# MartinMikkelsen/TensorTrainNumerics.jl

Measured on AMD Instinct MI355X. Metric: TT cores/sec for QTT Laplacian apply+round, d=30 rank-64, higher is better.
Workload: dtype f64

## Files before the change

### include/ttn.h

```cpp
#ifndef TTN_H
#define TTN_H

#include <stdint.h>

#ifdef __cplusplus
extern "C" {
#endif

#define TTN_OK                 0
#define TTN_ERR_DIMS          -1
#define TTN_ERR_BOND_INDEX    -2
#define TTN_ERR_SWEEPS        -3
#define TTN_ERR_CENTER        -4
#define TTN_ERR_CAPACITY      -5
#define TTN_ERR_ARG           -6
#define TTN_ERR_NOT_INIT      -7
#define TTN_ERR_UNSUPPORTED   -8
#define TTN_ERR_NO_CONVERGENCE -9
#define TTN_ERR_SINGULAR      -10

int         ttn_init(int device);
int         ttn_finalize(void);
const char* ttn_version(void);
const char* ttn_last_error_string(void);
// ... 120 lines not shown
int ttn_dot_pullback(ttn_tt_t a, ttn_tt_t b, const double* delta, ttn_tt_t abar, ttn_tt_t bbar, double* out);
int ttn_apply_pullback(ttn_tto_t A, ttn_tt_t x, ttn_tt_t ybar, ttn_tt_t xbar);
int ttn_tt_cores_axpby(const double* alpha, ttn_tt_t x, const double* beta, ttn_tt_t y);
int ttn_tt_cores_dot(ttn_tt_t x, ttn_tt_t y, double* out);

int ttn_hadamard(ttn_tt_t x, ttn_tt_t y, ttn_tt_t z);
int ttn_add(ttn_tt_t x, ttn_tt_t y, ttn_tt_t z);
int ttn_scale(double a, ttn_tt_t x, ttn_tt_t y);
int ttn_scale_batch(const double* a, ttn_tt_t x, ttn_tt_t y);
int ttn_orthogonalize(ttn_tt_t x, int64_t center, ttn_tt_t y);

int ttn_sv_capture(ttn_tt_t h, int enable);
int ttn_sv_get(ttn_tt_t h, int64_t b, int64_t step, double* out, int64_t cap, int64_t* n);

int ttn_timer_begin(void);
int ttn_timer_end(float* ms);
int ttn_event_record(int64_t slot);
int ttn_event_elapsed(int64_t slot_a, int64_t slot_b, float* ms);

int ttn_selftest_gemm(int64_t m, int64_t n, int64_t k, const double* A, const double* B, double* C, double alpha, double beta,
                      int ta, int tb);

int ttn_selftest_eig128(const double* G, int64_t n, int64_t r, int64_t nev, double* sig, double* X, int64_t* ticks_rc);
int ttn_selftest_sym_eig(int64_t N, int64_t k, const double* A, double* lam, double* Y);
int ttn_debug_ortho_state(int64_t b, int64_t* out4);

int ttn_apply_f64(int64_t d, const int64_t* dims,
                  const double* const* A_cores, const int64_t* A_rks,
                  const double* const* X_cores, const int64_t* X_rks,
                  double* const* Y_cores);
int ttn_dot_f64(int64_t d, const int64_t* dims,
                const double* const* A_cores, const int64_t* A_rks,
                const double* const* B_cores, const int64_t* B_rks, double* out);
int ttn_hadamard_f64(int64_t d, const int64_t* dims,
                     const double* const* X_cores, const int64_t* X_rks,
                     const double* const* Y_cores, const int64_t* Y_rks,
                     double* const* Z_cores);
int ttn_add_f64(int64_t d, const int64_t* dims,
                const double* const* X_cores, const int64_t* X_rks,
                const double* const* Y_cores, const int64_t* Y_rks,
                double* const* Z_cores);
int ttn_scale_f64(int64_t d, const int64_t* dims, double a,
                  const double* const* X_cores, const int64_t* X_rks, const int64_t* X_ot,
                  double* const* Y_cores, int64_t* Y_ot);
int ttn_orthogonalize_f64(int64_t d, const int64_t* dims,
                          const double* const* X_cores, const int64_t* X_rks, int64_t center,
// ... 48 lines not shown
```

### tensortrainnumerics.jl_amd/_lib.py

```python
from __future__ import annotations

import ctypes as C
import os
import subprocess

_HERE = os.path.dirname(os.path.abspath(__file__))
LIB_PATH = os.environ.get("TTN_LIB") or os.path.join(_HERE, "libttn_hip.so")
CSRC = os.path.join(_HERE, "csrc")
INCLUDE = os.path.join(os.path.dirname(_HERE), "include")

TTN_OK = 0
TTN_ERR_DIMS = -1
TTN_ERR_BOND_INDEX = -2
TTN_ERR_SWEEPS = -3
TTN_ERR_CENTER = -4
TTN_ERR_CAPACITY = -5
TTN_ERR_ARG = -6
TTN_ERR_NOT_INIT = -7
TTN_ERR_UNSUPPORTED = -8
TTN_ERR_NO_CONVERGENCE = -9
TTN_ERR_SINGULAR = -10

i64 = C.c_int64
p_i64 = C.POINTER(C.c_int64)
# ... 70 lines not shown
    "ttn_dmrg_linsolve": (C.c_int, [handle, handle, handle, handle, C.c_double, i64, p_i64, p_i64]),
    "ttn_dmrg_linsolve_it": (C.c_int, [handle, handle, handle, handle, C.c_double, i64, p_i64, p_i64, C.c_int, i64, C.c_double, i64]),
    "ttn_dmrg_cg_iterations": (C.c_int, [i64, p_i64]),
    "ttn_dmrg_eigsolve": (C.c_int, [handle, handle, handle, C.c_double, i64, p_i64, p_i64, C.c_int, i64, C.c_double, i64, i64, p_f64, p_i64]),
    "ttn_mals_eigsolve": (C.c_int, [handle, handle, handle, C.c_double, i64, p_i64, p_i64, C.c_int, i64, C.c_double, i64, i64, p_f64, p_i64]),
    "ttn_eigsolve_history_len": (C.c_int, [C.c_int, i64, i64, p_i64, p_i64]),
    "ttn_als_eigsolve": (C.c_int, [handle, handle, handle, i64, p_i64, p_i64, p_f64, i64, C.c_int, i64, C.c_double, i64, i64, p_f64]),
    "ttn_als_gen_eigsolve": (C.c_int, [handle, handle, handle, handle, i64, p_i64, p_i64, C.c_int, i64, i64, p_f64]),
    "ttn_eigsolve_stats": (C.c_int, [i64, p_i64, p_f64]),
    "ttn_tdvp_apply_h1": (C.c_int, [C.c_int, i64, i64, i64, i64, i64, i64, C.c_void_p, C.c_void_p, C.c_void_p, C.c_void_p, C.c_void_p, C.c_int]),
    "ttn_tdvp_apply_h0": (C.c_int, [C.c_int, i64, i64, i64, i64, C.c_void_p, C.c_void_p, C.c_void_p, C.c_void_p]),
    "ttn_tdvp_update_left_env": (C.c_int, [C.c_int, i64, i64, i64, i64, i64, i64, C.c_void_p, C.c_void_p, C.c_void_p, C.c_void_p, C.c_int]),
    "ttn_tdvp_update_right_env": (C.c_int, [C.c_int, i64, i64, i64, i64, i64, i64, C.c_void_p, C.c_void_p, C.c_void_p, C.c_void_p, C.c_int]),
    "ttn_tdvp_apply_h2": (C.c_int, [C.c_int, i64, i64, i64, i64, i64, i64, i64, i64, C.c_void_p, C.c_void_p, C.c_void_p, C.c_void_p, C.c_void_p, C.c_void_p, C.c_int]),
    "ttn_dense_qr": (C.c_int, [C.c_int, i64, i64, C.c_void_p, C.c_void_p, C.c_void_p]),
    "ttn_dense_svd": (C.c_int, [C.c_int, i64, i64, C.c_void_p, C.c_void_p, C.c_void_p, C.c_void_p]),
    "ttn_cross_maxvol": (C.c_int, [C.c_int, i64, i64, C.c_void_p, C.c_double, i64, C.c_void_p, C.c_void_p, C.c_void_p, p_i64]),
    "ttn_cross_points": (C.c_int, [C.c_int, C.c_int, i64, i64, i64, i64, i64, i64, C.c_void_p, C.c_void_p, C.c_void_p, i64, C.c_void_p,
                                   C.c_void_p, C.c_void_p, C.c_void_p]),
    "ttn_cross_eval": (C.c_int, [C.c_int, i64, i64, pp_f64, p_i64, p_i64, C.c_void_p, C.c_void_p, C.c_void_p, C.c_void_p, C.c_double,
                                 C.c_void_p]),
    "ttn_tdvp_contract_f64": (C.c_int, [C.c_int, C.c_int, i64, p_i64, C.c_void_p, C.c_void_p, C.c_void_p, C.c_void_p, C.c_void_p, C.c_void_p, C.c_int]),
    "ttn_selftest_eig128": (C.c_int, [C.c_void_p, i64, i64, i64, C.c_void_p, C.c_void_p, C.c_void_p]),
    "ttn_selftest_sym_eig": (C.c_int, [i64, i64, C.c_void_p, C.c_void_p, C.c_void_p]),
    "ttn_add": (C.c_int, [handle, handle, handle]),
    "ttn_scale": (C.c_int, [C.c_double, handle, handle]),
    "ttn_scale_batch": (C.c_int, [p_f64, handle, handle]),
    "ttn_orthogonalize": (C.c_int, [handle, i64, handle]),
    "ttn_sv_capture": (C.c_int, [handle, C.c_int]),
    "ttn_sv_get": (C.c_int, [handle, i64, i64, p_f64, i64, p_i64]),
    "ttn_timer_begin": (C.c_int, []),
    "ttn_timer_end": (C.c_int, [C.POINTER(C.c_float)]),
    "ttn_selftest_gemm": (C.c_int, [i64, i64, i64, p_f64, p_f64, p_f64, C.c_double, C.c_double, C.c_int, C.c_int]),
    "ttn_event_record": (C.c_int, [i64]),
    "ttn_event_elapsed": (C.c_int, [i64, i64, C.POINTER(C.c_float)]),
    "ttn_apply_f64": (C.c_int, [i64, p_i64, pp_f64, p_i64, pp_f64, p_i64, pp_f64]),
    "ttn_dot_f64": (C.c_int, [i64, p_i64, pp_f64, p_i64, pp_f64, p_i64, p_f64]),
    "ttn_hadamard_f64": (C.c_int, [i64, p_i64, pp_f64, p_i64, pp_f64, p_i64, pp_f64]),
    "ttn_add_f64": (C.c_int, [i64, p_i64, pp_f64, p_i64, pp_f64, p_i64, pp_f64]),
    "ttn_scale_f64": (C.c_int, [i64, p_i64, C.c_double, pp_f64, p_i64, p_i64, pp_f64, p_i64]),
    "ttn_orthogonalize_f64": (C.c_int, [i64, p_i64, pp_f64, p_i64, i64, pp_f64, p_i64, p_i64]),
    "ttn_compress_f64": (C.c_int, [i64, p_i64, pp_f64, p_i64, i64, C.c_double, i64]),
    "ttn_apply_compress_rank_bound": (C.c_int, [i64, p_i64, p_i64, p_i64, i64, i64, p_i64]),
    "ttn_apply_compress_f64": (C.c_int, [i64, p_i64, pp_f64, p_i64, pp_f64, p_i64, pp_f64, p_i64, i64, C.c_double, i64]),
    "ttn_bond_truncate_f64": (C.c_int, [i64, p_i64, pp_f64, p_i64, i64, i64, C.c_double]),
    "ttn_r_and_d_to_rks": (C.c_int, [i64, p_i64, i64, p_i64, i64, p_i64]),
# ... 121 lines not shown
```

### tensortrainnumerics.jl_amd/csrc/ttn_api.hip

```cpp
#include "../../include/ttn.h"
#include "ttn_common.h"
#include "ttn_stream_kernels.h"
#include "ttn_dense_kernels.h"
#include "ttn_dot_kernels.h"
#include "ttn_ortho_kernels.h"
#include "ttn_ortho512.h"
#include "ttn_ortho_ramp.h"
#include "ttn_hsvd_kernels.h"
#include "ttn_resite_kernels.h"
#include "ttn_als_kernels.h"
#include "ttn_als_grid.h"
#include "ttn_eigsolve_kernels.h"
#include "ttn_als_eig_kernels.h"
#include "ttn_eig_kernels.h"
#include "ttn_tdvp_kernels.h"
#include "ttn_densefact_kernels.h"
#include "ttn_cross_kernels.h"
#include "ttn_cross_batch_kernels.h"
#include "ttn_opalg_kernels.h"
#include "ttn_cplx_kernels.h"
#include "ttn_grid_kernels.h"
#include "ttn_grad_kernels.h"
#include "ttn_rect_kernels.h"
#include "ttn_step_kernels.h"

#include <algorithm>
#include <cmath>
#include <cstdio>
#include <cstring>
#include <cstdlib>
#include <mutex>
#include <set>
#include <string>
#include <vector>

extern "C" {
int ttn_wg512_init(void);
size_t ttn_wg512_compress_args_bytes(void);
int ttn_wg512_launch_compress(const void* args, size_t nbytes, int grid, hipStream_t stream);
int ttn_wg512_selftest_eig(const double* G, double* Vst, int n, int r, int nev, double* sig, double* Xout, long long* clk, hipStream_t stream);
int ttn_wg512_selftest_gemm(int m, int n, int k, double* A, double* B, double* C, double alpha, double beta, int ta, int tb, hipStream_t stream);
}

namespace {
std::set<struct ttn_tt_s*> g_live;
std::recursive_mutex g_mu;
bool g_init = false;
int g_device = -1;
hipStream_t g_stream = nullptr;
hipEvent_t g_ev0 = nullptr, g_ev1 = nullptr;
hipEvent_t g_launch_ev0 = nullptr, g_launch_ev1 = nullptr;
bool g_have_launch_ms = false;
size_t g_ortho_state_off = 0;
int g_ortho_state_batch = 0;
long long g_dense_plan[3] = {-1, 0, 0};
long long g_gather_plan[4] = {0, 0, 0, 0};
std::string g_err = "";
std::vector<hipEvent_t> g_slots;
std::vector<long long> g_xb_tab_host;
hipEvent_t g_xb_tab_ev = nullptr;

int fail(int code, const char* what) {
    g_err = what;
// ... 146 lines not shown

const char* ttn_version(void) { return "ttn-mi355x 0.1.0 (gfx950, fp64)"; }
const char* ttn_last_error_string(void) { return g_err.c_str(); }

int ttn_device_count(int* n) {
    if (!n) return fail(TTN_ERR_ARG, "null pointer");
    int c = 0;
    hipError_t e = hipGetDeviceCount(&c);
    if (e != hipSuccess) { *n = 0; return hipfail(e, "hipGetDeviceCount"); }
    *n = c;
    return TTN_OK;
}

int ttn_init(int device) {
    std::lock_guard<std::recursive_mutex> lk(g_mu);
    if (g_init && device == g_device) return TTN_OK;
    if (g_init) return fail(TTN_ERR_ARG, "ttn_init: already bound to another device (call ttn_finalize first)");
    HIPCHK(hipSetDevice(device));
    HIPCHK(hipStreamCreateWithFlags(&g_stream, hipStreamNonBlocking));
    for (hipEvent_t* e : {&g_ev0, &g_ev1, &g_launch_ev0, &g_launch_ev1}) HIPCHK(hipEventCreate(e));
    const struct { const void* fn; size_t lds; } lds_limits[] = {
        {(const void*)k_compress, COMPRESS_LDS_BYTES},
        {(const void*)k_selftest_eig128, COMPRESS_LDS_BYTES},
        {(const void*)k_mals_linsolve, COMPRESS_LDS_BYTES},
        {(const void*)k_als_linsolve, COMPRESS_LDS_BYTES},
        {(const void*)k_two_site_eig, COMPRESS_LDS_BYTES},
        {(const void*)k_als_eig, COMPRESS_LDS_BYTES},
        {(const void*)k_increase_ranks, COMPRESS_LDS_BYTES},
        {(const void*)k_ttv_decomp, COMPRESS_LDS_BYTES},
        {(const void*)k_split_sites, COMPRESS_LDS_BYTES},
        {(const void*)k_swap_chain, COMPRESS_LDS_BYTES},
        {(const void*)k_orthogonalize, ORTHO_LDS_BYTES},
        {(const void*)k_ortho512, O5_LDS_BYTES(TTN_MAX_D * 8)},
        {(const void*)k_dot_fused, DOT_LDS_BYTES(DOT_MAX_D)},
        {(const void*)k_grad_chain, DOT_LDS_BYTES(DOT_MAX_D)},
        {(const void*)k_selftest_gemm, sizeof(double) * GEMM_LDS_TOTAL},
        {(const void*)k_tdvp, TDVP_LDS_BYTES},
        {(const void*)k_lu_panel, LU_PANEL_LDS_BYTES},
        {(const void*)k_lu_trail, sizeof(double) * GEMM_LDS_TOTAL},
        {(const void*)k_cross_maxvol<false>, TTN_XV_LDS_BYTES},
        {(const void*)k_cross_maxvol<true>, TTN_XV_LDS_BYTES},
        {(const void*)k_zcompress, TTN_ZC_LDS_BYTES},
        {(const void*)k_cross_batch_site, TTN_XB_LDS_BYTES},
    };
    for (const auto& a : lds_limits) HIPCHK(hipFuncSetAttribute(a.fn, hipFuncAttributeMaxDynamicSharedMemorySize, (int)a.lds));
    { const int rc512 = ttn_wg512_init(); if (rc512) return hipfail((hipError_t)rc512, "ttn_wg512_init"); }
// ... 2401 lines not shown
    NEED_INIT();
    if (!A || !B || !C || m < 1 || n < 1 || k < 1) return fail(TTN_ERR_ARG, "bad argument");
    double *dA = nullptr, *dB = nullptr, *dC = nullptr;
    HIPCHK(hipMalloc((void**)&dA, sizeof(double) * m * k));
    HIPCHK(hipMalloc((void**)&dB, sizeof(double) * k * n));
    HIPCHK(hipMalloc((void**)&dC, sizeof(double) * m * n));
    HIPCHK(hipMemcpyAsync(dA, A, sizeof(double) * m * k, hipMemcpyHostToDevice, g_stream));
    HIPCHK(hipMemcpyAsync(dB, B, sizeof(double) * k * n, hipMemcpyHostToDevice, g_stream));
    HIPCHK(hipMemcpyAsync(dC, C, sizeof(double) * m * n, hipMemcpyHostToDevice, g_stream));
    if (getenv("TTN_WG512_SELFTEST") && atoi(getenv("TTN_WG512_SELFTEST"))) {
        const int rc512 = ttn_wg512_selftest_gemm((int)m, (int)n, (int)k, dA, dB, dC, alpha, beta, ta, tb, g_stream);
        if (rc512) return hipfail((hipError_t)rc512, "k_selftest_gemm (512-thread build)");
    } else {
    hipLaunchKernelGGL(k_selftest_gemm, dim3(1), dim3(TTN_WG), sizeof(double) * GEMM_LDS_TOTAL, g_stream, (int)m, (int)n, (int)k,
                       dA, dB, dC, alpha, beta, ta, tb);
    HIPCHK(hipGetLastError());
    }
    HIPCHK(hipMemcpyAsync(C, dC, sizeof(double) * m * n, hipMemcpyDeviceToHost, g_stream));
    HIPCHK(hipStreamSynchronize(g_stream));
    hipFree(dA); hipFree(dB); hipFree(dC);
    return TTN_OK;
}

int ttn_selftest_eig128(const double* G, int64_t n, int64_t r, int64_t nev, double* sig, double* X, int64_t* ticks_rc) {
    std::lock_guard<std::recursive_mutex> lk(g_mu);
    NEED_INIT();
    if (!G || !sig || !X || (n != 64 && n != 128) || r < 1 || r > 64 || nev < r || nev > n) return fail(TTN_ERR_ARG, "bad argument");
    double *dG = nullptr, *dV = nullptr, *dS = nullptr, *dX = nullptr;
    long long* dC = nullptr;
    HIPCHK(hipMalloc((void**)&dG, sizeof(double) * 128 * 128));
    HIPCHK(hipMalloc((void**)&dV, sizeof(double) * 128 * 128));
    HIPCHK(hipMalloc((void**)&dS, sizeof(double) * 128));
    HIPCHK(hipMalloc((void**)&dX, sizeof(double) * 128 * 64));
    HIPCHK(hipMalloc((void**)&dC, sizeof(long long) * 2));
    HIPCHK(hipMemcpyAsync(dG, G, sizeof(double) * n * n, hipMemcpyHostToDevice, g_stream));
    HIPCHK(hipMemsetAsync(dX, 0, sizeof(double) * 128 * 64, g_stream));
    if (getenv("TTN_WG512_SELFTEST") && atoi(getenv("TTN_WG512_SELFTEST"))) {
        const int rc512 = ttn_wg512_selftest_eig(dG, dV, (int)n, (int)r, (int)nev, dS, dX, dC, g_stream);
        if (rc512) return hipfail((hipError_t)rc512, "k_selftest_eig128 (512-thread build)");
    } else {
    hipLaunchKernelGGL(k_selftest_eig128, dim3(1), dim3(TTN_WG), COMPRESS_LDS_BYTES, g_stream, dG, dV, (int)n, (int)r, (int)nev, dS, dX, dC);
    HIPCHK(hipGetLastError());
    }
    long long hc[2] = {0, 0};
    HIPCHK(hipMemcpyAsync(sig, dS, sizeof(double) * nev, hipMemcpyDeviceToHost, g_stream));
    HIPCHK(hipMemcpyAsync(X, dX, sizeof(double) * 128 * r, hipMemcpyDeviceToHost, g_stream));
    HIPCHK(hipMemcpyAsync(hc, dC, sizeof(hc), hipMemcpyDeviceToHost, g_stream));
    HIPCHK(hipStreamSynchronize(g_stream));
    if (ticks_rc) { ticks_rc[0] = hc[0]; ticks_rc[1] = hc[1]; }
    hipFree(dG); hipFree(dV); hipFree(dS); hipFree(dX); hipFree(dC);
    return TTN_OK;
}

int ttn_selftest_sym_eig(int64_t N, int64_t k, const double* A, double* lam, double* Y) {
    std::lock_guard<std::recursive_mutex> lk(g_mu);
    if (!A || !lam || !Y || N < 1 || N > TTN_DENSE_LOCAL_MAX || k < 1 || k > std::min<int64_t>(N, TTN_NWAVES))
        return fail(TTN_ERR_ARG, "ttn_selftest_sym_eig: need 1 <= N <= 2048 and 1 <= k <= min(N, 16)");
    NEED_INIT();
    double *dA = nullptr, *dL = nullptr, *dY = nullptr, *dW = nullptr;
    HIPCHK(hipMalloc((void**)&dA, sizeof(double) * N * N));
    HIPCHK(hipMalloc((void**)&dL, sizeof(double) * k));
    HIPCHK(hipMalloc((void**)&dY, sizeof(double) * N * k));
    HIPCHK(hipMalloc((void**)&dW, sizeof(double) * (3 * N + 5 * N * k)));
    HIPCHK(hipMemcpyAsync(dA, A, sizeof(double) * N * N, hipMemcpyHostToDevice, g_stream));
    HIPCHK(hipMemsetAsync(dY, 0, sizeof(double) * N * k, g_stream));
    hipLaunchKernelGGL(k_selftest_sym_eig, dim3(1), dim3(TTN_WG), 0, g_stream, (int)N, (int)k, dA, dL, dY, dW);
    HIPCHK(hipGetLastError());
    HIPCHK(hipMemcpyAsync(lam, dL, sizeof(double) * k, hipMemcpyDeviceToHost, g_stream));
    HIPCHK(hipMemcpyAsync(Y, dY, sizeof(double) * N * k, hipMemcpyDeviceToHost, g_stream));
    HIPCHK(hipStreamSynchronize(g_stream));
    hipFree(dA); hipFree(dL); hipFree(dY); hipFree(dW);
    return TTN_OK;
}

// ... 1218 lines not shown
```

### tensortrainnumerics.jl_amd/csrc/ttn_eig_kernels.h

```cpp
#pragma once
#include "ttn_dense_kernels.h"

#define EIG_N 128
template <int J>
__device__ __forceinline__ void fmac_bcast(double& a, double w, double s_) {
    asm volatile("v_fmac_f64_dpp %0, %1, %2 row_newbcast:%3 row_mask:0xf bank_mask:0xf" : "+v"(a) : "v"(w), "v"(s_), "n"(J));
}
#define EIG_BCAST16(M) M(0) M(1) M(2) M(3) M(4) M(5) M(6) M(7) M(8) M(9) M(10) M(11) M(12) M(13) M(14) M(15)
#define EIG_TAIL TTN_LDS_IMG

__device__ __forceinline__ void lds_barrier() { asm volatile("s_waitcnt lgkmcnt(0)\n\ts_barrier" ::: "memory"); }
__device__ __forceinline__ double wave64_sum_mfma(double v) {
    v = grp_sum(v);
    v += dpp_mov_f64<0x124>(v);
    v += dpp_mov_f64<0x128>(v);
    return v;
}
__device__ __forceinline__ double readlane_f64(double v, int idx) {
    union { double d; int i[2]; } u, r;
    u.d = v;
    r.i[0] = __builtin_amdgcn_readlane(u.i[0], idx);
    r.i[1] = __builtin_amdgcn_readlane(u.i[1], idx);
    return r.d;
}
// ... 100 lines not shown
            const double nvi = -vL[i], nwi = -wL[i];
            asm volatile("s_nop 1");
#define EIG_UP(j) fmac_bcast<j>(a[j], wreg[0], nvi); fmac_bcast<j>(a[j], vreg[0], nwi);
            EIG_BCAST16(EIG_UP)
#undef EIG_UP
            if constexpr (NH == 2) {
#define EIG_UP(j) fmac_bcast<j>(a[16 + j], wreg[1], nvi); fmac_bcast<j>(a[16 + j], vreg[1], nwi);
                EIG_BCAST16(EIG_UP)
#undef EIG_UP
            }
            if (i == k + 2) {
#pragma unroll
                for (int j = 0; j < CW; ++j) xn_w[CW * c + j] = a[j];
            }
        }
    }
    __syncthreads();
    if (actv && i == N - 2 && c == NC - 1) { dg[N - 2] = a[CW - 2]; e[N - 2] = a[CW - 1]; }
    if (actv && i == N - 1 && c == NC - 1) { dg[N - 1] = a[CW - 1]; }
    __syncthreads();
}

template <int N>
__device__ __forceinline__ int sturm_count(const double (&dreg)[N / 16], const double (&ereg)[N / 16], double x, bool& zero) {
    double pc = 1.0, pp = 0.0;
    const double nx = -x, one = 1.0;
    int cnt = 0;
    bool z = false;
    unsigned int prev = 0;
#pragma unroll
    for (int g = 0; g < N / 16; ++g) {
        unsigned int bits = 0;
#define EIG_ST(j) {                                                                                               \
            double dmx = nx;                                                                                      \
            fmac_bcast<j>(dmx, dreg[g], one);                                         \
            double pn = dmx * pc;                                                                                 \
            fmac_bcast<j>(pn, ereg[g], pp);                        \
            z |= (pn == 0.0);                                                                                     \
            bits = __builtin_amdgcn_alignbit(bits, (unsigned int)(__double_as_longlong(pn) >> 32), 31);           \
            pp = pc; pc = pn; }
        EIG_BCAST16(EIG_ST)
#undef EIG_ST
        const unsigned int seq = (prev << 16) | (bits & 0xffffu);
        cnt += __popc((seq ^ (seq >> 1)) & 0xffffu);
        prev = bits & 1u;
        const double ap = fabs(pc);
        if (ap < 0x1p-400 || ap > 0x1p400) {
            const double sc = (ap < 1.0) ? 0x1p500 : 0x1p-500;
            pc *= sc; pp *= sc;
        }
    }
    zero = z;
    return cnt;
}
__device__ __noinline__ int sturm_count_guarded(const lds_f64* de, double x, int n) {
    double pc = 1.0, pp = 0.0;
    int cnt = 0;
    for (int i = 0; i < n; ++i) {
        double pn = fma(de[2 * i] - x, pc, de[2 * i + 1] * pp);
        if (pn == 0.0) pn = copysign(DBL_MIN, -pc);
        cnt += (int)(((unsigned long long)(__double_as_longlong(pn) ^ __double_as_longlong(pc))) >> 63);
        pp = pc; pc = pn;
        const double ap = fabs(pc);
        if (ap < 0x1p-400 || ap > 0x1p400) { const double sc = (ap < 1.0) ? 0x1p500 : 0x1p-500; pc *= sc; pp *= sc; }
    }
    return cnt;
}

template <int N, int TL>
__device__ void wg_bisect(int nev, double* lds) {
    lds_f64* L = (lds_f64*)lds;
    lds_f64 *dg = L + EIG_TAIL, *e = dg + 128, *lam = dg + 256;
    lds_f64* e2 = L;
    const int tid = threadIdx.x;
    lds_f64* de = L + 256;
    for (int t = tid; t < N; t += TTN_WG) { e2[t] = (t < N - 1) ? e[t] * e[t] : 0.0; de[2 * t] = dg[t]; de[2 * t + 1] = (t > 0) ? -(e[t - 1] * e[t - 1]) : 0.0; }
    __syncthreads();
    if (tid < 64) {
        double glo_ = 1e300, ghi_ = -1e300, emax_ = 0.0;
        for (int t = tid; t < N; t += 64) {
            const double rad = ((t > 0) ? fabs(e[t - 1]) : 0.0) + ((t < N - 1) ? fabs(e[t]) : 0.0);
            glo_ = fmin(glo_, dg[t] - rad); ghi_ = fmax(ghi_, dg[t] + rad);
            emax_ = fmax(emax_, e2[t]);
        }
        glo_ = -wave_max(-glo_); ghi_ = wave_max(ghi_); emax_ = wave_max(emax_);
        if (tid == 0) { e2[128] = glo_; e2[129] = ghi_; e2[130] = emax_; }
    }
    __syncthreads();
    double glo = e2[128], ghi = e2[129];
    const double emax = e2[130];
    const double span = fmax(fabs(glo), fabs(ghi));
    glo -= 2.0 * DBL_EPSILON * span * N; ghi += 2.0 * DBL_EPSILON * span * N;
    const double pivmin = DBL_MIN * fmax(1.0, emax);
    double dreg[N / 16], ereg[N / 16];
#pragma unroll
    for (int g = 0; g < N / 16; ++g) { dreg[g] = de[2 * (16 * g + (tid & 15))]; ereg[g] = de[2 * (16 * g + (tid & 15)) + 1]; }
    asm volatile("s_nop 1");
    for (int g0 = 0; g0 < nev; g0 += TTN_WG / TL) {
        const int gi = g0 + tid / TL, sub = tid % TL;
        const bool act = gi < nev;
        const int jasc = N - 1 - (act ? gi : 0);
        double lo = glo, hi = ghi;
        for (int round = 0; round < 64; ++round) {
            const double wdt = hi - lo;
            const bool done = !(wdt > 2.0 * DBL_EPSILON * fmax(fabs(lo), fabs(hi)) + 2.0 * pivmin);
            if (__syncthreads_and(done || !act)) break;
            const double x = lo + wdt * ((double)(sub + 1) / (double)(TL + 1));
            const bool wave_act = g0 + (tid & ~63) / TL < nev;
            bool zero = false;
            int cnt = wave_act ? sturm_count<N>(dreg, ereg, x, zero) : 0;
            if (zero) cnt = sturm_count_guarded(de, x, N);
            int nf = (cnt <= jasc) ? 1 : 0;
#pragma unroll
            for (int m = 1; m < TL; m <<= 1) nf += __shfl_xor(nf, m);
            if (!done) {
                const double nlo = (nf > 0) ? lo + wdt * ((double)nf / (double)(TL + 1)) : lo;
                const double nhi = (nf < TL) ? lo + wdt * ((double)(nf + 1) / (double)(TL + 1)) : hi;
                lo = nlo; hi = nhi;
            }
        }
        if (act && sub == 0) lam[gi] = 0.5 * (lo + hi);
    }
    __syncthreads();
}

template <int N>
struct EigDm {
    static constexpr bool IN_LDS = 2 * N * 64 <= TTN_LDS_IMG;
    typedef __attribute__((address_space(1))) double gdouble;
    lds_f64* l;
    gdouble* g;
    __device__ __forceinline__ double ld(int idx) const { if constexpr (IN_LDS) return l[idx]; else return g[idx]; }
    __device__ __forceinline__ void st(int idx, double v) const { if constexpr (IN_LDS) l[idx] = v; else g[idx] = v; }
};
template <int N>
__device__ void wg_twisted(int r, double* lds, int* tw , lds_f64* zn , double* Dmg) {
    lds_f64* L = (lds_f64*)lds;
    lds_f64 *dg = L + EIG_TAIL, *e = dg + 128, *lam = dg + 256;
    lds_f64* Dp = L;
    EigDm<N> Dm;
    Dm.l = L + N * 64; Dm.g = (typename EigDm<N>::gdouble*)(unsigned long long)Dmg;
    const int tid = threadIdx.x, lane = tid & 63, wave = tid >> 6;
    double emax = 0.0;
    for (int t = 0; t < N - 1; ++t) emax = fmax(emax, e[t] * e[t]);
    const double pivmin = DBL_MIN * fmax(1.0, emax);
// ... 60 lines not shown
                for (int i0 = 0; i0 < N - 1; i0 += 8) {
                    double dm[8];
#pragma unroll
                    for (int t = 0; t < 8; ++t) dm[t] = (i0 + t + 1 < N) ? Dm.ld((i0 + t + 1) * 64 + lane) : 1.0;
#pragma unroll
                    for (int t = 0; t < 8; ++t) {
                        const int i = i0 + t;
                        if (i >= kb && i < N - 1) {
                            z = -(e[i] * fast_rcp(dm[t])) * z;
                            Dm.st((i + 1) * 64 + lane, z);
                            nrm = fma(z, z, nrm);
                        }
                    }
                }
            }
            if (act) zn[64 + lane] = nrm;
        }
    }
    __syncthreads();
    if (tid < 64 && tid < r) zn[tid] = 1.0 / sqrt(1.0 + zn[tid] + zn[64 + tid]);
    __syncthreads();
}

template <int N>
__device__ __noinline__ int wg_eig_n(const double* Gg, int ldg, double* Vst, int r, int nev, double* sig, double* lds, int* iwork ,
                                     double* dwork ) {
    Gg = unip(Gg); Vst = unip(Vst); sig = unip(sig); lds = unip(lds); iwork = unip(iwork); dwork = unip(dwork);
    r = uni32(r); nev = uni32(nev); ldg = uni32(ldg);
    constexpr int RPL = N / 16;
    lds_f64* L = (lds_f64*)lds;
    lds_f64 *lam = L + EIG_TAIL + 256, *beta = L + EIG_TAIL + 384;
    const int tid = threadIdx.x, lane = tid & 63, wave = tid >> 6;
    __builtin_amdgcn_s_setprio(TTN_EIG_PRIO);
    wg_tridiag<N>(Gg, ldg, Vst, lds);
    if (nev <= 32) wg_bisect<N, 8>(nev, lds);
    else wg_bisect<N, 4>(nev, lds);
    int bad = 0;
    for (int j = tid; j < nev; j += TTN_WG) { const double l = lam[j]; sig[j] = (l > 0.0) ? sqrt(l) : 0.0; bad |= (j < r) && !(l > 0.0); }
    if (__syncthreads_or(bad)) {
        __builtin_amdgcn_s_setprio(0); TTN_SETPRIO_BASE();
        return 1;
    }
    wg_twisted<N>(r, lds, iwork, (lds_f64*)dwork, const_cast<double*>(Gg));
    lds_f64* Dp = L;
    EigDm<N> Dm;
    Dm.l = L + N * 64; Dm.g = (typename EigDm<N>::gdouble*)(unsigned long long)Gg;
    const int rc = (lane & 3) | ((lane >> 4) << 2), col0 = 8 * (wave & 7) + 2 * ((lane >> 2) & 3);
    double z[2][RPL];
#pragma unroll
    for (int cc = 0; cc < 2; ++cc) {
        const int col = col0 + cc;
        const int kb = (col < r) ? iwork[col] : 0;
        const double zn = (col < r) ? ((lds_f64*)dwork)[col] : 0.0;
#pragma unroll
        for (int t = 0; t < RPL; ++t) {
            const int row = RPL * rc + t;
            const double v = (row < kb) ? Dp[row * 64 + col] : ((row == kb) ? 1.0 : Dm.ld(row * 64 + col));
            z[cc][t] = v * zn;
        }
// ... 35 lines not shown
        }
    }
    __syncthreads();
    __builtin_amdgcn_s_setprio(0); TTN_SETPRIO_BASE();
    return 0;
}
__device__ int wg_eig128(const double* Gg, double* Vst, int r, int nev, double* sig, double* lds, int* iwork, double* dwork) {
    return wg_eig_n<128>(Gg, 128, Vst, r, nev, sig, lds, iwork, dwork);
}
__device__ int wg_eig64(const double* Gg, int ldg, double* Vst, int r, int nev, double* sig, double* lds, int* iwork, double* dwork) {
    return wg_eig_n<64>(Gg, ldg, Vst, r, nev, sig, lds, iwork, dwork);
}

__global__ void TTN_KERNEL_BOUNDS k_selftest_eig128(const double* G, double* Vst, int n, int r, int nev, double* sig, double* Xout, long long* clk) {
    extern __shared__ double lds[];
    int* iwork = reinterpret_cast<int*>(lds + GEMM_LDS_TOTAL + 32);
    double* dwork = lds + GEMM_LDS_TOTAL + 32 + 64;
    const long long t0 = (long long)__builtin_amdgcn_s_memtime();
    const int rc = (n == 64) ? wg_eig_n<64>(G, 64, Vst, r, nev, sig, lds, iwork, dwork) : wg_eig_n<128>(G, 128, Vst, r, nev, sig, lds, iwork, dwork);
    const long long t1 = (long long)__builtin_amdgcn_s_memtime();
    if (threadIdx.x == 0) { clk[0] = t1 - t0; clk[1] = rc; }
    if (rc == 0) for (int e = threadIdx.x; e < 128 * r; e += TTN_WG) Xout[e] = lds[e];
}
```

### tensortrainnumerics.jl_amd/csrc/ttn_wg512.hip

```cpp
#include <hip/hip_runtime.h>
#include <stdint.h>
#include <float.h>
#include <string.h>

#define TTN_WG 512
namespace ttn_wg512 {
#include "ttn_common.h"
#include "ttn_dense_kernels.h"
#include "ttn_eig_kernels.h"
}

extern "C" {

int ttn_wg512_init(void) {
    hipError_t e;
    if ((e = hipFuncSetAttribute(reinterpret_cast<const void*>(ttn_wg512::k_compress), hipFuncAttributeMaxDynamicSharedMemorySize, (int)COMPRESS_LDS_BYTES)) != hipSuccess) return (int)e;
    if ((e = hipFuncSetAttribute(reinterpret_cast<const void*>(ttn_wg512::k_selftest_eig128), hipFuncAttributeMaxDynamicSharedMemorySize, (int)COMPRESS_LDS_BYTES)) != hipSuccess) return (int)e;
    if ((e = hipFuncSetAttribute(reinterpret_cast<const void*>(ttn_wg512::k_selftest_gemm), hipFuncAttributeMaxDynamicSharedMemorySize, (int)COMPRESS_LDS_BYTES)) != hipSuccess) return (int)e;
    return 0;
}

size_t ttn_wg512_compress_args_bytes(void) { return sizeof(ttn_wg512::CompressArgs); }
size_t ttn_wg512_lds_bytes(void) { return COMPRESS_LDS_BYTES; }

int ttn_wg512_launch_compress(const void* args, size_t nbytes, int grid, hipStream_t stream) {
    if (nbytes != sizeof(ttn_wg512::CompressArgs)) return (int)hipErrorInvalidValue;
    ttn_wg512::CompressArgs P;
    memcpy(&P, args, sizeof(P));
    hipLaunchKernelGGL(ttn_wg512::k_compress, dim3(grid), dim3(TTN_WG), COMPRESS_LDS_BYTES, stream, P);
    return (int)hipGetLastError();
}

int ttn_wg512_selftest_eig(const double* G, double* Vst, int n, int r, int nev, double* sig, double* Xout, long long* clk, hipStream_t stream) {
    hipLaunchKernelGGL(ttn_wg512::k_selftest_eig128, dim3(1), dim3(TTN_WG), COMPRESS_LDS_BYTES, stream, G, Vst, n, r, nev, sig, Xout, clk);
    return (int)hipGetLastError();
}
int ttn_wg512_selftest_gemm(int m, int n, int k, double* A, double* B, double* C, double alpha, double beta, int ta, int tb, hipStream_t stream) {
    hipLaunchKernelGGL(ttn_wg512::k_selftest_gemm, dim3(1), dim3(TTN_WG), COMPRESS_LDS_BYTES, stream, m, n, k, A, B, C, alpha, beta, ta, tb);
    return (int)hipGetLastError();
}

}
```

Measured before the change: 603,700.

## Accelerate tridiagonal bisection with coarse Sturm table and interpolated probe placement

The workgroup bisection eigensolver first evaluates a 256-point Sturm-count table over the Gershgorin interval. Each eigenvalue then starts from the bracketing table cell instead of the full interval. Within the bracket, probes are clustered around a secant or quadratic root estimate, built from the tracked mantissa and exponent of the Sturm recurrence's final pivot. A closing bisection replay reproduces the original bracket sequence and only calls Sturm counts where a probe falls inside the refined bracket, aiming to cut the number of Sturm passes in the SVD used by rounding. It also adds a statistics-collecting selftest kernel, at the cost of more register and LDS use and more complex control flow.

```diff
diff --git a/include/ttn.h b/include/ttn.h
--- a/include/ttn.h
+++ b/include/ttn.h
@@ -166,6 +166,7 @@
                       int ta, int tb);
 
 int ttn_selftest_eig128(const double* G, int64_t n, int64_t r, int64_t nev, double* sig, double* X, int64_t* ticks_rc);
+int ttn_selftest_eig128_ex(const double* G, int64_t n, int64_t r, int64_t nev, double* sig, double* X, int64_t* info);
 int ttn_selftest_sym_eig(int64_t N, int64_t k, const double* A, double* lam, double* Y);
 int ttn_debug_ortho_state(int64_t b, int64_t* out4);
 
diff --git a/tensortrainnumerics.jl_amd/_lib.py b/tensortrainnumerics.jl_amd/_lib.py
--- a/tensortrainnumerics.jl_amd/_lib.py
+++ b/tensortrainnumerics.jl_amd/_lib.py
@@ -116,6 +116,7 @@
                                  C.c_void_p]),
     "ttn_tdvp_contract_f64": (C.c_int, [C.c_int, C.c_int, i64, p_i64, C.c_void_p, C.c_void_p, C.c_void_p, C.c_void_p, C.c_void_p, C.c_void_p, C.c_int]),
     "ttn_selftest_eig128": (C.c_int, [C.c_void_p, i64, i64, i64, C.c_void_p, C.c_void_p, C.c_void_p]),
+    "ttn_selftest_eig128_ex": (C.c_int, [C.c_void_p, i64, i64, i64, C.c_void_p, C.c_void_p, C.c_void_p]),
     "ttn_selftest_sym_eig": (C.c_int, [i64, i64, C.c_void_p, C.c_void_p, C.c_void_p]),
     "ttn_add": (C.c_int, [handle, handle, handle]),
     "ttn_scale": (C.c_int, [C.c_double, handle, handle]),
diff --git a/tensortrainnumerics.jl_amd/csrc/ttn_api.hip b/tensortrainnumerics.jl_amd/csrc/ttn_api.hip
--- a/tensortrainnumerics.jl_amd/csrc/ttn_api.hip
+++ b/tensortrainnumerics.jl_amd/csrc/ttn_api.hip
@@ -39,6 +39,7 @@
 size_t ttn_wg512_compress_args_bytes(void);
 int ttn_wg512_launch_compress(const void* args, size_t nbytes, int grid, hipStream_t stream);
 int ttn_wg512_selftest_eig(const double* G, double* Vst, int n, int r, int nev, double* sig, double* Xout, long long* clk, hipStream_t stream);
+int ttn_wg512_selftest_eig_ex(const double* G, double* Vst, int n, int r, int nev, double* sig, double* Xout, long long* clk, hipStream_t stream);
 int ttn_wg512_selftest_gemm(int m, int n, int k, double* A, double* B, double* C, double alpha, double beta, int ta, int tb, hipStream_t stream);
 }
 
@@ -231,6 +232,7 @@
     const struct { const void* fn; size_t lds; } lds_limits[] = {
         {(const void*)k_compress, COMPRESS_LDS_BYTES},
         {(const void*)k_selftest_eig128, COMPRESS_LDS_BYTES},
+        {(const void*)k_selftest_eig128_ex, COMPRESS_LDS_BYTES},
         {(const void*)k_mals_linsolve, COMPRESS_LDS_BYTES},
         {(const void*)k_als_linsolve, COMPRESS_LDS_BYTES},
         {(const void*)k_two_site_eig, COMPRESS_LDS_BYTES},
@@ -2678,7 +2680,7 @@
     return TTN_OK;
 }
 
-int ttn_selftest_eig128(const double* G, int64_t n, int64_t r, int64_t nev, double* sig, double* X, int64_t* ticks_rc) {
+static int selftest_eig128_impl(const double* G, int64_t n, int64_t r, int64_t nev, double* sig, double* X, int64_t* words, int nwords) {
     std::lock_guard<std::recursive_mutex> lk(g_mu);
     NEED_INIT();
     if (!G || !sig || !X || (n != 64 && n != 128) || r < 1 || r > 64 || nev < r || nev > n) return fail(TTN_ERR_ARG, "bad argument");
@@ -2688,24 +2690,34 @@
     HIPCHK(hipMalloc((void**)&dV, sizeof(double) * 128 * 128));
     HIPCHK(hipMalloc((void**)&dS, sizeof(double) * 128));
     HIPCHK(hipMalloc((void**)&dX, sizeof(double) * 128 * 64));
-    HIPCHK(hipMalloc((void**)&dC, sizeof(long long) * 2));
+    HIPCHK(hipMalloc((void**)&dC, sizeof(long long) * 4));
     HIPCHK(hipMemcpyAsync(dG, G, sizeof(double) * n * n, hipMemcpyHostToDevice, g_stream));
     HIPCHK(hipMemsetAsync(dX, 0, sizeof(double) * 128 * 64, g_stream));
+    HIPCHK(hipMemsetAsync(dC, 0, sizeof(long long) * 4, g_stream));
+    const bool ex = nwords == 4;
     if (getenv("TTN_WG512_SELFTEST") && atoi(getenv("TTN_WG512_SELFTEST"))) {
-        const int rc512 = ttn_wg512_selftest_eig(dG, dV, (int)n, (int)r, (int)nev, dS, dX, dC, g_stream);
+        const int rc512 = ex ? ttn_wg512_selftest_eig_ex(dG, dV, (int)n, (int)r, (int)nev, dS, dX, dC, g_stream)
+                             : ttn_wg512_selftest_eig(dG, dV, (int)n, (int)r, (int)nev, dS, dX, dC, g_stream);
         if (rc512) return hipfail((hipError_t)rc512, "k_selftest_eig128 (512-thread build)");
     } else {
-    hipLaunchKernelGGL(k_selftest_eig128, dim3(1), dim3(TTN_WG), COMPRESS_LDS_BYTES, g_stream, dG, dV, (int)n, (int)r, (int)nev, dS, dX, dC);
-    HIPCHK(hipGetLastError());
-    }
-    long long hc[2] = {0, 0};
+    if (ex) hipLaunchKernelGGL(k_selftest_eig128_ex, dim3(1), dim3(TTN_WG), COMPRESS_LDS_BYTES, g_stream, dG, dV, (int)n, (int)r, (int)nev, dS, dX, dC);
+    else hipLaunchKernelGGL(k_selftest_eig128, dim3(1), dim3(TTN_WG), COMPRESS_LDS_BYTES, g_stream, dG, dV, (int)n, (int)r, (int)nev, dS, dX, dC);
+    HIPCHK(hipGetLastError());
+    }
+    long long hc[4] = {0, 0, 0, 0};
     HIPCHK(hipMemcpyAsync(sig, dS, sizeof(double) * nev, hipMemcpyDeviceToHost, g_stream));
     HIPCHK(hipMemcpyAsync(X, dX, sizeof(double) * 128 * r, hipMemcpyDeviceToHost, g_stream));
     HIPCHK(hipMemcpyAsync(hc, dC, sizeof(hc), hipMemcpyDeviceToHost, g_stream));
     HIPCHK(hipStreamSynchronize(g_stream));
-    if (ticks_rc) { ticks_rc[0] = hc[0]; ticks_rc[1] = hc[1]; }
+    if (words) for (int i = 0; i < nwords; ++i) words[i] = hc[i];
     hipFree(dG); hipFree(dV); hipFree(dS); hipFree(dX); hipFree(dC);
     return TTN_OK;
+}
+int ttn_selftest_eig128(const double* G, int64_t n, int64_t r, int64_t nev, double* sig, double* X, int64_t* ticks_rc) {
+    return selftest_eig128_impl(G, n, r, nev, sig, X, ticks_rc, 2);
+}
+int ttn_selftest_eig128_ex(const double* G, int64_t n, int64_t r, int64_t nev, double* sig, double* X, int64_t* info) {
+    return selftest_eig128_impl(G, n, r, nev, sig, X, info, 4);
 }
 
 int ttn_selftest_sym_eig(int64_t N, int64_t k, const double* A, double* lam, double* Y) {
diff --git a/tensortrainnumerics.jl_amd/csrc/ttn_eig_kernels.h b/tensortrainnumerics.jl_amd/csrc/ttn_eig_kernels.h
--- a/tensortrainnumerics.jl_amd/csrc/ttn_eig_kernels.h
+++ b/tensortrainnumerics.jl_amd/csrc/ttn_eig_kernels.h
@@ -146,10 +146,10 @@
 }
 
 template <int N>
-__device__ __forceinline__ int sturm_count(const double (&dreg)[N / 16], const double (&ereg)[N / 16], double x, bool& zero) {
+__device__ __forceinline__ int sturm_count(const double (&dreg)[N / 16], const double (&ereg)[N / 16], double x, bool& zero, double& mant, int& expo) {
     double pc = 1.0, pp = 0.0;
     const double nx = -x, one = 1.0;
-    int cnt = 0;
+    int cnt = 0, sh = 0;
     bool z = false;
     unsigned int prev = 0;
 #pragma unroll
@@ -170,11 +170,16 @@
         prev = bits & 1u;
         const double ap = fabs(pc);
         if (ap < 0x1p-400 || ap > 0x1p400) {
-            const double sc = (ap < 1.0) ? 0x1p500 : 0x1p-500;
+            const bool up = ap < 1.0;
+            const double sc = up ? 0x1p500 : 0x1p-500;
             pc *= sc; pp *= sc;
+            sh += up ? -500 : 500;
         }
     }
     zero = z;
+    int ex = 0;
+    mant = frexp(pc, &ex);
+    expo = sh + ex;
     return cnt;
 }
 __device__ __noinline__ int sturm_count_guarded(const lds_f64* de, double x, int n) {
@@ -191,13 +196,21 @@
     return cnt;
 }
 
-template <int N, int TL>
+#define EIG_NCOARSE 256
+#define EIG_FSTOP 8.0
+#define EIG_UNUSABLE (-(1 << 30))
+#define EIG_STATS_SLOT (EIG_TAIL + 511)
+template <int N, int TL, bool STATS>
 __device__ void wg_bisect(int nev, double* lds) {
     lds_f64* L = (lds_f64*)lds;
     lds_f64 *dg = L + EIG_TAIL, *e = dg + 128, *lam = dg + 256;
     lds_f64* e2 = L;
     const int tid = threadIdx.x;
     lds_f64* de = L + 256;
+    lds_f64* tm = L + 512;
+    lds_i32* tc = (lds_i32*)(L + 768);
+    lds_i32* te = (lds_i32*)(L + 896);
+    int* stats = (int*)(lds + EIG_STATS_SLOT);
     for (int t = tid; t < N; t += TTN_WG) { e2[t] = (t < N - 1) ? e[t] * e[t] : 0.0; de[2 * t] = dg[t]; de[2 * t + 1] = (t > 0) ? -(e[t - 1] * e[t - 1]) : 0.0; }
     __syncthreads();
     if (tid < 64) {
@@ -216,35 +229,164 @@
     const double span = fmax(fabs(glo), fabs(ghi));
     glo -= 2.0 * DBL_EPSILON * span * N; ghi += 2.0 * DBL_EPSILON * span * N;
     const double pivmin = DBL_MIN * fmax(1.0, emax);
+    const double gw = ghi - glo;
     double dreg[N / 16], ereg[N / 16];
 #pragma unroll
     for (int g = 0; g < N / 16; ++g) { dreg[g] = de[2 * (16 * g + (tid & 15))]; ereg[g] = de[2 * (16 * g + (tid & 15)) + 1]; }
     asm volatile("s_nop 1");
+    if (tid < EIG_NCOARSE) {
+        const double x = glo + gw * ((double)(tid + 1) / (double)(EIG_NCOARSE + 1));
+        bool zero = false;
+        double m;
+        int ex;
+        int cnt = sturm_count<N>(dreg, ereg, x, zero, m, ex);
+        if (zero) cnt = sturm_count_guarded(de, x, N);
+        if (zero || !(fabs(m) >= 0.5 && fabs(m) < 1.0)) ex = EIG_UNUSABLE;
+        tm[tid] = m; tc[tid] = cnt; te[tid] = ex;
+    }
+    __syncthreads();
+    auto tab_x = [&](int i) { return (i <= 0) ? glo : ((i > EIG_NCOARSE) ? ghi : glo + gw * ((double)i / (double)(EIG_NCOARSE + 1))); };
+    auto tab_c = [&](int i) { return (i <= 0) ? 0 : ((i > EIG_NCOARSE) ? N : tc[i - 1]); };
+    auto tab_e = [&](int i) { return (i <= 0 || i > EIG_NCOARSE) ? EIG_UNUSABLE : te[i - 1]; };
+    auto tab_m = [&](int i) { return (i <= 0 || i > EIG_NCOARSE) ? 0.0 : tm[i - 1]; };
+    const int sub = tid % TL;
+    const double frac = (double)(sub + 1) / (double)(TL + 1);
+    const int half = TL / 2, steps = (sub < half) ? half - 1 - sub : sub - half;
+    const double mult = ((sub < half) ? -1.0 : 1.0) * (double)(1 << ((TL == 4 ? 4 : 2) * steps));
     for (int g0 = 0; g0 < nev; g0 += TTN_WG / TL) {
-        const int gi = g0 + tid / TL, sub = tid % TL;
+        const int gi = g0 + tid / TL;
         const bool act = gi < nev;
         const int jasc = N - 1 - (act ? gi : 0);
-        double lo = glo, hi = ghi;
-        for (int round = 0; round < 64; ++round) {
+        int ta = 0, tb = EIG_NCOARSE + 1;
+#pragma unroll
+        for (int it = 0; it < 9; ++it) {
+            if (tb - ta > 1) {
+                const int mid = (ta + tb) >> 1;
+                if (tc[mid - 1] <= jasc) ta = mid; else tb = mid;
+            }
+        }
+        double lo = tab_x(ta), hi = tab_x(ta + 1), mlo = tab_m(ta), mhi = tab_m(ta + 1);
+        int clo = tab_c(ta), chi = tab_c(ta + 1), elo = tab_e(ta), ehi = tab_e(ta + 1);
+        double xo = 0.0, mo = 0.0;
+        int eo = EIG_UNUSABLE;
+        {
+            const int lt = (ta >= 1 && tab_e(ta - 1) != EIG_UNUSABLE) ? ta - 1 : -1;
+            const int rt = (ta + 2 <= EIG_NCOARSE + 1 && tab_e(ta + 2) != EIG_UNUSABLE) ? ta + 2 : -1;
+            const int pick = (lt >= 0 && (rt < 0 || tab_c(lt) == clo || tab_c(rt) != chi)) ? lt : rt;
+            if (pick >= 0) { xo = tab_x(pick); mo = tab_m(pick); eo = tab_e(pick); }
+        }
+        bool forced = false;
+        int myrounds = 1;
+        for (int round = 0; round < 128; ++round) {
             const double wdt = hi - lo;
-            const bool done = !(wdt > 2.0 * DBL_EPSILON * fmax(fabs(lo), fabs(hi)) + 2.0 * pivmin);
+            const double tolw = 2.0 * DBL_EPSILON * fmax(fabs(lo), fabs(hi)) + 2.0 * pivmin;
+            const bool done = !(wdt > EIG_FSTOP * tolw);
             if (__syncthreads_and(done || !act)) break;
-            const double x = lo + wdt * ((double)(sub + 1) / (double)(TL + 1));
-            const bool wave_act = g0 + (tid & ~63) / TL < nev;
+            double x = lo + wdt * frac;
+            bool placed = false;
+            if (!forced && chi - clo == 1 && elo != EIG_UNUSABLE && ehi != EIG_UNUSABLE && ((mlo < 0.0) != (mhi < 0.0))) {
+                int E = max(elo, ehi);
+                if (eo != EIG_UNUSABLE) E = max(E, eo);
+                const double flo = ldexp(mlo, max(elo - E, -2000)), fhi = ldexp(mhi, max(ehi - E, -2000));
+                const double s = lo + wdt * (flo * fast_rcp(flo - fhi));
+                double est = s, dqs = wdt;
+                if (eo != EIG_UNUSABLE) {
+                    const double fo = ldexp(mo, max(eo - E, -2000));
+                    const double whi = (flo * fo) * fast_rcp((fhi - flo) * (fhi - fo));
+                    const double wo = (flo * fhi) * fast_rcp((fo - flo) * (fo - fhi));
+                    const double q = lo + (wdt * whi + (xo - lo) * wo);
+                    if (q > lo && q < hi) est = q;
+                    dqs = fabs(q - s);
+                }
+                if (!(dqs < wdt)) dqs = wdt;
+                const double delta = fmin(fmax(2.0 * dqs, 0.5 * tolw), 0.125 * wdt);
+                const double c = est + mult * delta;
+                if (c > lo && c < hi) x = c;
+                placed = true;
+            }
+            const bool wave_act = __builtin_amdgcn_ballot_w64(act && !done) != 0ull;
             bool zero = false;
-            int cnt = wave_act ? sturm_count<N>(dreg, ereg, x, zero) : 0;
+            double m = 0.0;
+            int ex = EIG_UNUSABLE, cnt = 0;
+            if (wave_act) {
+                asm volatile("s_nop 1");
+                cnt = sturm_count<N>(dreg, ereg, x, zero, m, ex);
+                if constexpr (STATS) { if ((tid & 63) == 0) atomicAdd(stats + 1, 1); }
+            }
             if (zero) cnt = sturm_count_guarded(de, x, N);
-            int nf = (cnt <= jasc) ? 1 : 0;
-#pragma unroll
-            for (int m = 1; m < TL; m <<= 1) nf += __shfl_xor(nf, m);
+            if (zero || !(fabs(m) >= 0.5 && fabs(m) < 1.0)) ex = EIG_UNUSABLE;
+            double xl = -INFINITY, ml = 0.0, xr = INFINITY, mr = 0.0;
+            int el = EIG_UNUSABLE, er = EIG_UNUSABLE;
+            if (eo != EIG_UNUSABLE && xo < lo) { xl = xo; ml = mo; el = eo; }
+            if (eo != EIG_UNUSABLE && xo > hi) { xr = xo; mr = mo; er = eo; }
+            double nlo = lo, nmlo = mlo, nhi = hi, nmhi = mhi;
+            int nclo = clo, nelo = elo, nchi = chi, nehi = ehi;
+#pragma unroll
+            for (int t = 0; t < TL; ++t) {
+                const double xt = __shfl(x, t, TL), mt = __shfl(m, t, TL);
+                const int ct = __shfl(cnt, t, TL), et = __shfl(ex, t, TL);
+                if (ct <= jasc) {
+                    if (xt > nlo) { xl = nlo; ml = nmlo; el = nelo; nlo = xt; nclo = ct; nmlo = mt; nelo = et; }
+                    else if (xt > xl) { xl = xt; ml = mt; el = et; }
+                } else {
+                    if (xt < nhi) { xr = nhi; mr = nmhi; er = nehi; nhi = xt; nchi = ct; nmhi = mt; nehi = et; }
+                    else if (xt < xr) { xr = xt; mr = mt; er = et; }
+                }
+            }
             if (!done) {
-                const double nlo = (nf > 0) ? lo + wdt * ((double)nf / (double)(TL + 1)) : lo;
-                const double nhi = (nf < TL) ? lo + wdt * ((double)(nf + 1) / (double)(TL + 1)) : hi;
-                lo = nlo; hi = nhi;
-            }
-        }
-        if (act && sub == 0) lam[gi] = 0.5 * (lo + hi);
-    }
+                lo = nlo; clo = nclo; mlo = nmlo; elo = nelo; hi = nhi; chi = nchi; mhi = nmhi; ehi = nehi;
+                const bool left = el != EIG_UNUSABLE && (er == EIG_UNUSABLE || lo - xl <= xr - hi);
+                xo = left ? xl : xr; mo = left ? ml : mr; eo = left ? el : er;
+                forced = placed && (hi - lo) > wdt * (1.0 / (double)(TL + 1));
+                ++myrounds;
+            }
+        }
+        double plo = glo, phi = ghi;
+        for (int rr = 0; rr < 64; ++rr) {
+            const double pw = phi - plo;
+            const bool pdone = !act || !(pw > 2.0 * DBL_EPSILON * fmax(fabs(plo), fabs(phi)) + 2.0 * pivmin);
+            if (__builtin_amdgcn_ballot_w64(!pdone) == 0ull) break;
+            const double x = plo + pw * frac;
+            const bool amb = !pdone && x > lo && x < hi;
+            bool below = x <= lo;
+            if (__builtin_amdgcn_ballot_w64(amb) != 0ull) {
+                bool zero = false;
+                double m;
+                int ex;
+                asm volatile("s_nop 1");
+                int cnt = sturm_count<N>(dreg, ereg, x, zero, m, ex);
+                if (zero) cnt = sturm_count_guarded(de, x, N);
+                below = cnt <= jasc;
+                if constexpr (STATS) { if ((tid & 63) == 0) atomicAdd(stats + 1, 1); }
+#pragma unroll
+                for (int t = 0; t < TL; ++t) {
+                    const double xt = __shfl(x, t, TL);
+                    const int bt = __shfl((int)below, t, TL);
+                    if (!pdone && xt > lo && xt < hi) { if (bt) lo = xt; else hi = xt; }
+                }
+                if constexpr (STATS) {
+                    int ag = amb ? 1 : 0;
+#pragma unroll
+                    for (int mk = 1; mk < TL; mk <<= 1) ag |= __shfl_xor(ag, mk);
+                    if (ag) ++myrounds;
+                }
+            }
+            int nf = below ? 1 : 0;
+#pragma unroll
+            for (int mk = 1; mk < TL; mk <<= 1) nf += __shfl_xor(nf, mk);
+            if (!pdone) {
+                double f0 = 0.0, f1 = 0.0;
+#pragma unroll
+                for (int j = 1; j <= TL; ++j) { if (nf == j) f0 = (double)j / (double)(TL + 1); if (nf + 1 == j) f1 = (double)j / (double)(TL + 1); }
+                const double nlo = (nf > 0) ? plo + pw * f0 : plo;
+                const double nhi = (nf < TL) ? plo + pw * f1 : phi;
+                plo = nlo; phi = nhi;
+            }
+        }
+        if (act && sub == 0) lam[gi] = 0.5 * (plo + phi);
+        if constexpr (STATS) { if (act && sub == 0) atomicMax(stats, myrounds); }
+    }
+    if constexpr (STATS) { if (tid == 0) atomicAdd(stats + 1, 4); }
     __syncthreads();
 }
 
@@ -351,7 +493,7 @@
     __syncthreads();
 }
 
-template <int N>
+template <int N, bool STATS = false>
 __device__ __noinline__ int wg_eig_n(const double* Gg, int ldg, double* Vst, int r, int nev, double* sig, double* lds, int* iwork ,
                                      double* dwork ) {
     Gg = unip(Gg); Vst = unip(Vst); sig = unip(sig); lds = unip(lds); iwork = unip(iwork); dwork = unip(dwork);
@@ -362,8 +504,8 @@
     const int tid = threadIdx.x, lane = tid & 63, wave = tid >> 6;
     __builtin_amdgcn_s_setprio(TTN_EIG_PRIO);
     wg_tridiag<N>(Gg, ldg, Vst, lds);
-    if (nev <= 32) wg_bisect<N, 8>(nev, lds);
-    else wg_bisect<N, 4>(nev, lds);
+    if (nev <= 32) wg_bisect<N, 8, STATS>(nev, lds);
+    else wg_bisect<N, 4, STATS>(nev, lds);
     int bad = 0;
     for (int j = tid; j < nev; j += TTN_WG) { const double l = lam[j]; sig[j] = (l > 0.0) ? sqrt(l) : 0.0; bad |= (j < r) && !(l > 0.0); }
     if (__syncthreads_or(bad)) {
@@ -445,3 +587,19 @@
     if (threadIdx.x == 0) { clk[0] = t1 - t0; clk[1] = rc; }
     if (rc == 0) for (int e = threadIdx.x; e < 128 * r; e += TTN_WG) Xout[e] = lds[e];
 }
+
+__global__ void TTN_KERNEL_BOUNDS k_selftest_eig128_ex(const double* G, double* Vst, int n, int r, int nev, double* sig, double* Xout, long long* clk) {
+    extern __shared__ double lds[];
+    int* iwork = reinterpret_cast<int*>(lds + GEMM_LDS_TOTAL + 32);
+    double* dwork = lds + GEMM_LDS_TOTAL + 32 + 64;
+    int* stats = reinterpret_cast<int*>(lds + EIG_STATS_SLOT);
+    if (threadIdx.x == 0) { stats[0] = 0; stats[1] = 0; }
+    __syncthreads();
+    const long long t0 = (long long)__builtin_amdgcn_s_memtime();
+    const int rc = (n == 64) ? wg_eig_n<64, true>(G, 64, Vst, r, nev, sig, lds, iwork, dwork) : wg_eig_n<128, true>(G, 128, Vst, r, nev, sig, lds, iwork, dwork);
+    const long long t1 = (long long)__builtin_amdgcn_s_memtime();
+    __syncthreads();
+    if (threadIdx.x == 0) { clk[0] = t1 - t0; clk[1] = rc; clk[2] = stats[0]; clk[3] = stats[1]; }
+    __syncthreads();
+    if (rc == 0) for (int e = threadIdx.x; e < 128 * r; e += TTN_WG) Xout[e] = lds[e];
+}
diff --git a/tensortrainnumerics.jl_amd/csrc/ttn_wg512.hip b/tensortrainnumerics.jl_amd/csrc/ttn_wg512.hip
--- a/tensortrainnumerics.jl_amd/csrc/ttn_wg512.hip
+++ b/tensortrainnumerics.jl_amd/csrc/ttn_wg512.hip
@@ -16,6 +16,7 @@
     hipError_t e;
     if ((e = hipFuncSetAttribute(reinterpret_cast<const void*>(ttn_wg512::k_compress), hipFuncAttributeMaxDynamicSharedMemorySize, (int)COMPRESS_LDS_BYTES)) != hipSuccess) return (int)e;
     if ((e = hipFuncSetAttribute(reinterpret_cast<const void*>(ttn_wg512::k_selftest_eig128), hipFuncAttributeMaxDynamicSharedMemorySize, (int)COMPRESS_LDS_BYTES)) != hipSuccess) return (int)e;
+    if ((e = hipFuncSetAttribute(reinterpret_cast<const void*>(ttn_wg512::k_selftest_eig128_ex), hipFuncAttributeMaxDynamicSharedMemorySize, (int)COMPRESS_LDS_BYTES)) != hipSuccess) return (int)e;
     if ((e = hipFuncSetAttribute(reinterpret_cast<const void*>(ttn_wg512::k_selftest_gemm), hipFuncAttributeMaxDynamicSharedMemorySize, (int)COMPRESS_LDS_BYTES)) != hipSuccess) return (int)e;
     return 0;
 }
@@ -35,6 +36,10 @@
     hipLaunchKernelGGL(ttn_wg512::k_selftest_eig128, dim3(1), dim3(TTN_WG), COMPRESS_LDS_BYTES, stream, G, Vst, n, r, nev, sig, Xout, clk);
     return (int)hipGetLastError();
 }
+int ttn_wg512_selftest_eig_ex(const double* G, double* Vst, int n, int r, int nev, double* sig, double* Xout, long long* clk, hipStream_t stream) {
+    hipLaunchKernelGGL(ttn_wg512::k_selftest_eig128_ex, dim3(1), dim3(TTN_WG), COMPRESS_LDS_BYTES, stream, G, Vst, n, r, nev, sig, Xout, clk);
+    return (int)hipGetLastError();
+}
 int ttn_wg512_selftest_gemm(int m, int n, int k, double* A, double* B, double* C, double alpha, double beta, int ta, int tb, hipStream_t stream) {
     hipLaunchKernelGGL(ttn_wg512::k_selftest_gemm, dim3(1), dim3(TTN_WG), COMPRESS_LDS_BYTES, stream, m, n, k, A, B, C, alpha, beta, ta, tb);
     return (int)hipGetLastError();
```

New measurement: 603,900, median of 3. About the same (+0.0%).
